# SmoothKen/knn-svc

Measured on AMD Instinct MI355X. Metric: audio-sec converted/sec (xRT) end-to-end, cold target pool, higher is better.
Workload: dtype f32; 1 GPU; north-star point per rank: 30 s source vs 10 min target pool (20 x 30 s), ckpt_type=mix, post_opt_0.2, cold (pool encoded inside the step); seeded random weights of WavLM-Large (6 layers executed) and the 22.9 M-param generator; nq=1500, np_per_rank=30000, wavlm_batch_chunks=32, pipeline_depth=2

## Files before the change

knn_svc_amd/csrc/gemm2_core.h:

```cpp
#pragma once
#include "common.h"

typedef _Float16 f16x8 __attribute__((ext_vector_type(8)));
typedef _Float16 f16x2_t __attribute__((ext_vector_type(2)));
typedef float f32x2_t __attribute__((ext_vector_type(2)));
typedef unsigned g2_u32x4 __attribute__((ext_vector_type(4)));
typedef unsigned g2_u32x2 __attribute__((ext_vector_type(2)));

constexpr float KN_F16X2_A_SCALE = 16.0f;

__device__ __forceinline__ void f16x2_split4(f32x4 v, float scale, g2_u32x2& hi, g2_u32x2& lo) {
    f32x2_t a = {v[0], v[1]}, b = {v[2], v[3]};
    a *= scale; b *= scale;
    const f16x2_t ha = __builtin_convertvector(a, f16x2_t), hb = __builtin_convertvector(b, f16x2_t);
    const f32x2_t ra = a - __builtin_convertvector(ha, f32x2_t), rb = b - __builtin_convertvector(hb, f32x2_t);
    const f16x2_t la = __builtin_convertvector(ra, f16x2_t), lb = __builtin_convertvector(rb, f16x2_t);
    hi = (g2_u32x2){__builtin_bit_cast(unsigned, ha), __builtin_bit_cast(unsigned, hb)};
    lo = (g2_u32x2){__builtin_bit_cast(unsigned, la), __builtin_bit_cast(unsigned, lb)};
}

typedef __attribute__((address_space(3))) char g2_lds_c;
typedef __attribute__((address_space(3))) g2_u32x4 g2_lds_u4;
typedef __attribute__((address_space(3))) g2_u32x2 g2_lds_u2;

#ifdef KN_WHATIF_NOMFMA
#define KN_F16X2_MMA3(C, FA, FB) C[0] += (float)FA[1][0] * (float)FB[0][0] + (float)FA[0][1] * (float)FB[1][1];
#else
#define KN_F16X2_MMA3(C, FA, FB)                                                                               \
    C = __builtin_amdgcn_mfma_f32_32x32x16_f16(FA[1], FB[0], C, 0, 0, 0);               \
    C = __builtin_amdgcn_mfma_f32_32x32x16_f16(FA[0], FB[1], C, 0, 0, 0);                                      \
    C = __builtin_amdgcn_mfma_f32_32x32x16_f16(FA[0], FB[0], C, 0, 0, 0);
#endif
#define KN_F16X2_SLAB_MMA(A, B)                                                                                \
    _Pragma("unroll") for (int ks = 0; ks < 2; ++ks) {                                                        \
        f16x8 fa[TM][2], fb[TN][2];                                                                            \
        _Pragma("unroll") for (int i = 0; i < TM; ++i)                                                        \
            _Pragma("unroll") for (int p = 0; p < 2; ++p)                                                     \
                fa[i][p] = __builtin_bit_cast(f16x8, *(const g2_lds_u4*)(A + i * 32 * PITCH + p * 64 + ks * 32)); \
        _Pragma("unroll") for (int j = 0; j < TN; ++j)                                                        \
            _Pragma("unroll") for (int p = 0; p < 2; ++p)                                                     \
                fb[j][p] = __builtin_bit_cast(f16x8, *(const g2_lds_u4*)(B + j * 32 * PITCH + p * 64 + ks * 32)); \
        _Pragma("unroll") for (int i = 0; i < TM; ++i)                                                        \
            _Pragma("unroll") for (int j = 0; j < TN; ++j) {                                                  \
                f32x16 c = acc[i][j];                                                                          \
                KN_F16X2_MMA3(c, fa[i], fb[j])                                                                 \
                acc[i][j] = c;                                                                                 \
            }                                                                                                  \
    }
#define KN_SPLIT_B_LOAD(RB, SLAB)                                                                              \
    { const int sl_ = SLAB; bload.begin(sl_); _Pragma("unroll") for (int j = 0; j < B_P; ++j) RB[j] = bload(sl_, j, rb_desc); }
#define KN_SPLIT_B_STAGE(RB, BOFF)                                                                             \
    _Pragma("unroll") for (int j = 0; j < B_P; ++j) {                                                         \
        const int q = tid + 256 * j;                                                                          \
        if (B_PIECES % 256 == 0 || q < B_PIECES) *(g2_lds_u4*)(lds + BOFF + (q >> 3) * PITCH + (q & 7) * 16) = RB[j]; \
    }

__host__ __device__ __forceinline__ bool quad_order_swap(long gx, long gy) {
    const long gx8 = (gx + 7) / 8 * 8, gy8 = (gy + 7) / 8 * 8;
    return (gx8 - gx) * 16 > gx8 && (gx8 - gx) * gy8 > (gy8 - gy) * gx8;
}
__host__ __device__ __forceinline__ bool quad_order_linear(long gx, long gy) {
    const long gx8 = (gx + 7) / 8 * 8, gy8 = (gy + 7) / 8 * 8;
    return (gx8 - gx) * 16 > gx8 && (gy8 - gy) * 16 > gy8;
}
__host__ __device__ __forceinline__ long quad_order_ids(long gx, long gy) {
    if (quad_order_linear(gx, gy)) return gx * gy;
    return quad_order_swap(gx, gy) ? (gy + 7) / 8 * 8 * gx : (gx + 7) / 8 * 8 * gy;
}
__device__ __forceinline__ bool quad_order_decode(int L, int gx, int gy, int& mt, int& nt, int rot = 0) {
    if (quad_order_linear(gx, gy)) { mt = L % gx; nt = L / gx; return true; }
    const bool sw = quad_order_swap(gx, gy);
    const int ga = sw ? gy : gx, gb = sw ? gx : gy;
    const int ga8 = (ga + 7) / 8 * 8;
    constexpr int CW = 4;
    const int full = (gb / CW) * CW * ga8;
    int c0, cw;
    if (L < full) { c0 = (L / (CW * ga8)) * CW; cw = CW; L -= (c0 / CW) * CW * ga8; }
    else { c0 = (gb / CW) * CW; cw = gb - c0; L -= full; }
    const int grp = L / (8 * cw), rem = L - grp * 8 * cw;
    const int at = grp * 8 + ((rem + rot) & 7), bt = c0 + (rem >> 3);
    mt = sw ? bt : at; nt = sw ? at : bt;
    return at < ga;
}

__host__ __device__ __forceinline__ bool patch_order_plain(long gx, long gy) { return gy == 1 && gx % 8 != 0; }
__host__ __device__ __forceinline__ long patch_order_ids(long gx, long gy) {
    return (patch_order_plain(gx, gy) ? gx : (gx + 7) / 8 * 8) * gy;
}
template <int BM, int BN>
__device__ __forceinline__ bool patch_order_decode(int plain, int m, int n, int& m0, int& n0) {
    const int gy = (n + BN - 1) / BN;
    const int gx8 = (int)gridDim.x / gy;
    constexpr int CW = 8;
    int L = blockIdx.x;
    const int full = (gy / CW) * CW * gx8;
    int c0, cw;
    if (L < full) { c0 = (L / (CW * gx8)) * CW; cw = CW; L -= (c0 / CW) * CW * gx8; }
    else { c0 = (gy / CW) * CW; cw = gy - c0; L -= full; }
    const int grp = L / (8 * cw), rem = L - grp * 8 * cw;
    m0 = plain ? (int)blockIdx.x * BM : (grp * 8 + ((rem + (int)blockIdx.z) & 7)) * BM;
    n0 = plain ? 0 : (c0 + (rem >> 3)) * BN;
    return m0 < m;
}

#ifdef KN_QUAD_PROF
__device__ long long kn_quad_prof_buf[8192 * 4];
#endif

template <int BM_, int BN_, int WM_, int WN_, int TM_, int TN_>
struct Gemm2Tile : Acc32<WN_, TM_, TN_> {
    typedef f32x16 acc_t;
    static constexpr int NR = 16;
    static constexpr int BM = BM_, BN = BN_, WM = WM_, WN = WN_, TM = TM_, TN = TN_;
    static constexpr int BK = 32, PITCH = 144, THREADS = 256;
    static_assert(WM * WN == 4 && WM * TM * 32 == BM && WN * TN * 32 == BN, "tile shape");
    static constexpr int A_F4 = BM / 32;
    static constexpr int B_PIECES = BN * 8;
    static constexpr int B_P = (B_PIECES + 255) / 256;
    static constexpr int LDS_BYTES = (BM + BN) * PITCH;

    __device__ __forceinline__ static void split_store(g2_lds_c* dst, f32x4 v, float a_scale) {
        g2_u32x2 hi, lo;
        f16x2_split4(v, a_scale, hi, lo);
        *(g2_lds_u2*)(dst) = hi;
        *(g2_lds_u2*)(dst + 64) = lo;
    }

    template <bool A2 = false, class ALoad, class BLoad, class RA, class RB>
    __device__ __forceinline__ static void mainloop(float* lds_generic, int nk, ALoad& aload, BLoad& bload,
                                                    f32x16 (&acc)[TM][TN], RA ra_desc, RB rb_desc, float a_scale) {
        g2_lds_c* lds = (g2_lds_c*)lds_generic;
        const int tid = threadIdx.x;
        const int a_st = (tid >> 3) * PITCH + (tid & 7) * (A2 ? 16 : 8);
        const int lane = tid & 63, wave = tid >> 6;
        const int wm = wave / WN, wn = wave % WN;
        const int li = lane & 31, lh = lane >> 5;
        const int a_frag = (wm * TM * 32 + li) * PITCH + lh * 16;
        const int b_frag = BM * PITCH + (wn * TN * 32 + li) * PITCH + lh * 16;

        f32x4 ra[A_F4];
        g2_u32x4 rb[B_P];
#define KN_STAGE2()                                                                                               \
    {                                                                                                            \
        _Pragma("unroll") for (int j = 0; j < A_F4; ++j) {                                                       \
            if constexpr (A2) *(g2_lds_u4*)(lds + a_st + 32 * j * PITCH) = __builtin_bit_cast(g2_u32x4, ra[j]);   \
            else split_store(lds + a_st + 32 * j * PITCH, aload.finish(ra[j]), a_scale);                         \
        }                                                                                                        \
        KN_SPLIT_B_STAGE(rb, BM * PITCH)                                                                         \
    }
        aload.begin(0); bload.begin(0);
#pragma unroll
        for (int j = 0; j < A_F4; ++j) ra[j] = aload(0, j, ra_desc);
#pragma unroll
        for (int j = 0; j < B_P; ++j) rb[j] = bload(0, j, rb_desc);
        KN_STAGE2();
        __syncthreads();

        for (int kt = 0; kt < nk; ++kt) {
            const bool more = (kt + 1 < nk);
            if (more) {
                aload.begin(kt + 1); bload.begin(kt + 1);
#pragma unroll
                for (int j = 0; j < A_F4; ++j) ra[j] = aload(kt + 1, j, ra_desc);
#pragma unroll
                for (int j = 0; j < B_P; ++j) rb[j] = bload(kt + 1, j, rb_desc);
            }
            KN_F16X2_SLAB_MMA(lds + a_frag, lds + b_frag)
            __syncthreads();
            if (more) KN_STAGE2();
            __syncthreads();
        }
#undef KN_STAGE2
    }
};

struct Gemm2QuadS {
    typedef f32x4 acc_t;
    static constexpr int NR = 4;
    static constexpr int BM = 256, BN = 256, WM = 2, WN = 2, TM = 8, TN = 8;
    static constexpr int EPI_TN = 4;
    static constexpr int ROW = 128, NW = 4, THREADS = 256;
    static constexpr int A_P = BM * ROW / 1024 / NW, B_P = BN * ROW / 1024 / NW;
    static_assert(A_P == 8 && B_P == 8, "schedule below is written for 8 + 8 pieces");
    static constexpr int BOFF = BM * ROW;
    static constexpr int STAGE = (BM + BN) * ROW;
    static constexpr int EPI_BYTES = NW * 32 * (EPI_TN * 32 + 4) * 4;
    static constexpr int LDS_BYTES = 2 * STAGE > EPI_BYTES ? 2 * STAGE : EPI_BYTES;
    static constexpr int OOB_OFF = 0x40000000;

    typedef __attribute__((address_space(3))) char lds_c;
    typedef __attribute__((address_space(3))) g2_u32x4 lds_u4;

    template <class RowOff, class Step, class RA, class RB>
    __device__ __forceinline__ static void mainloop(float* lds_generic, int nk, RowOff a_row_off, Step a_step, RA ra_desc,
                                                    RB rb_desc, int N, int K, int m0, int n0, f32x4 (&acc)[TM][TN]) {
        lds_c* lds = (lds_c*)lds_generic;
        const int tid = threadIdx.x, lane = tid & 63, wave = __builtin_amdgcn_readfirstlane(tid >> 6);
        const int wm = wave / WN, wn = wave % WN;
        const int a_row = (wm * 128 + (lane & 15)) * ROW;
        const int b_row = BOFF + (wn * 128 + (lane & 15)) * ROW;
        int x_off[2];
#pragma unroll
        for (int p = 0; p < 2; ++p) x_off[p] = ((p * 4 + (lane >> 4)) ^ (lane & 7)) * 16;
        int a_src[A_P], b_src[B_P];
        const int row_bytes = (K / 32) * 128;
#pragma unroll
        for (int t = 0; t < A_P; ++t) {
            const int row = (wave * A_P + t) * 8 + (lane >> 3);
            const int ro = a_row_off(m0 + row);
            a_src[t] = ro == OOB_OFF ? OOB_OFF : ro + (lane & 7) * 16;
        }
#pragma unroll
        for (int t = 0; t < B_P; ++t) {
            const int row = (wave * B_P + t) * 8 + (lane >> 3);
            b_src[t] = (n0 + row < N) ? (n0 + row) * row_bytes + (lane & 7) * 16 : OOB_OFF;
        }
        const int st_dst = wave * 8 * 1024 + (lane >> 3) * ROW + (((lane & 7) ^ (lane >> 3)) * 16);
        int ua = 0;
        int a_issued = 0, b_issued = 0;
        g2_u32x4 st[8];
#define KN_S_LOAD_A(T) { st[T] = __builtin_amdgcn_raw_buffer_load_b128(ra_desc, a_src[T] + ua, 0, 0); }
#define KN_S_LOAD_B(T) { st[T] = __builtin_amdgcn_raw_buffer_load_b128(rb_desc, b_src[T], b_issued * 128, 0); }
#define KN_S_WRITE(T, OFF) { *(lds_u4*)(lds + (OFF) + st_dst + (T) * 1024) = st[T]; }
        f16x8 fa[2][4][2], fb[2][4][2];
#define KN_S_READ_A(SET, STG, II, I) { _Pragma("unroll") for (int p = 0; p < 2; ++p) fa[SET][I][p] = __builtin_bit_cast(f16x8, *(const lds_u4*)(lds + (STG) + a_row + ((II) * 4 + (I)) * 16 * ROW + x_off[p])); }
#define KN_S_READ_B(SET, STG, JJ, J) { _Pragma("unroll") for (int p = 0; p < 2; ++p) fb[SET][J][p] = __builtin_bit_cast(f16x8, *(const lds_u4*)(lds + (STG) + b_row + ((JJ) * 4 + (J)) * 16 * ROW + x_off[p])); }
#define KN_S_MFMA1(C, A, B) asm volatile("v_mfma_f32_16x16x32_f16 %0, %1, %2, %0" : "+a"(C) : "v"(A), "v"(B));
#define KN_S_MFMA(AS, BS, I, J)                                                                                           \
    {                                                                                                                     \
        KN_S_MFMA1(acc[(AS) * 4 + (I)][(BS) * 4 + (J)], fa[AS][I][1], fb[BS][J][0])                 \
        KN_S_MFMA1(acc[(AS) * 4 + (I)][(BS) * 4 + (J)], fa[AS][I][0], fb[BS][J][1])                                       \
        KN_S_MFMA1(acc[(AS) * 4 + (I)][(BS) * 4 + (J)], fa[AS][I][0], fb[BS][J][0])                                       \
    }
        ua = a_step(0);
#pragma unroll
        for (int t = 0; t < 8; ++t) KN_S_LOAD_A(t)
        a_issued = 1;
#pragma unroll
        for (int t = 0; t < 8; ++t) KN_S_WRITE(t, 0)
#pragma unroll
        for (int t = 0; t < 8; ++t) KN_S_LOAD_B(t)
        b_issued = 1;
#pragma unroll
        for (int t = 0; t < 8; ++t) KN_S_WRITE(t, BOFF)
        if (nk > 1) {
            ua = a_step(1);
#pragma unroll
            for (int t = 0; t < 8; ++t) KN_S_LOAD_A(t)
            a_issued = 2;
        }
        __builtin_amdgcn_s_waitcnt(0xC07F);
        __builtin_amdgcn_s_barrier();
#ifdef KN_QUAD_PROF
        if (threadIdx.x == 0 && blockIdx.x < 8192) kn_quad_prof_buf[blockIdx.x * 4 + 1] = (long long)__builtin_amdgcn_s_memrealtime();
#endif
#pragma unroll
        for (int i = 0; i < 4; ++i) KN_S_READ_A(0, 0, 0, i)
#pragma unroll
        for (int j = 0; j < 4; ++j) KN_S_READ_B(0, 0, 0, j)

#define KN_S_SLAB(FB, HN, ML)                                                                                             \
    {                                                                                                                     \
        constexpr int cstg = (FB) * STAGE, nstg = (1 - (FB)) * STAGE;              \
                                                                                                     \
        _Pragma("unroll") for (int t = 0; t < 16; ++t) {                                                                  \
            KN_S_MFMA(0, FB, t >> 2, t & 3)                                                                               \
            __builtin_amdgcn_sched_barrier(0);                                                                            \
            if (t < 8) { if (t < 4) KN_S_READ_B(1 - (FB), cstg, 1 - (FB), t) }                                            \
            else if (HN) KN_S_WRITE(t - 8, nstg)                                                                          \
            __builtin_amdgcn_sched_barrier(0);                                                                            \
        }                                                                                                                 \
                                                                                                   \
        _Pragma("unroll") for (int t = 0; t < 16; ++t) {                                                                  \
            KN_S_MFMA(0, 1 - (FB), t >> 2, t & 3)                                                                         \
            __builtin_amdgcn_sched_barrier(0);                                                                            \
            if (t < 8) { if (HN) KN_S_LOAD_B(t) }                                                                         \
            else if (t < 12) KN_S_READ_A(1, cstg, 1, t - 8)                                                               \
            __builtin_amdgcn_sched_barrier(0);                                                                            \
        }                                                                                                                 \
        if (HN) ++b_issued;                                                                                               \
        if (ML) ua = a_step(a_issued);                                                                                    \
                                                                                                   \
        _Pragma("unroll") for (int t = 0; t < 16; ++t) {                                                                  \
            KN_S_MFMA(1, 1 - (FB), t >> 2, t & 3)                                                                         \
            __builtin_amdgcn_sched_barrier(0);                                                                            \
            if (t >= 8) {                                                                                                 \
                if (HN) KN_S_WRITE(t - 8, nstg + BOFF)                                                                    \
                if (ML) KN_S_LOAD_A(t - 8)                                                                                \
            }                                                                                                             \
            __builtin_amdgcn_sched_barrier(0);                                                                            \
        }                                                                                                                 \
        if (ML) ++a_issued;                                                                                               \
        if (HN) { __builtin_amdgcn_s_waitcnt(0xC07F); __builtin_amdgcn_s_barrier(); }                                     \
                     \
        _Pragma("unroll") for (int t = 0; t < 16; ++t) {                                                                  \
            KN_S_MFMA(1, FB, t >> 2, t & 3)                                                                               \
            __builtin_amdgcn_sched_barrier(0);                                                                            \
            if (HN) {                                                                                                     \
                if (t < 4) KN_S_READ_A(0, nstg, 0, t)                                                                     \
                else if (t >= 8 && t < 12) KN_S_READ_B(1 - (FB), nstg, 1 - (FB), t - 8)                                   \
            }                                                                                                             \
            __builtin_amdgcn_sched_barrier(0);                                                                            \
        }                                                                                                                 \
    }
        int s = 0;
        for (; s + 1 < nk; s += 2) {
            KN_S_SLAB(0, true, true)
            KN_S_SLAB(1, true, true)
        }
        if (s < nk) KN_S_SLAB(0, true, true)
#undef KN_S_SLAB
#undef KN_S_MFMA
#undef KN_S_MFMA1
#undef KN_S_READ_A
#undef KN_S_READ_B
#undef KN_S_WRITE
#undef KN_S_LOAD_A
#undef KN_S_LOAD_B
    }

    __device__ __forceinline__ static int acc_row(int wave, int lane, int i, int r) { return (wave / WN) * 128 + i * 16 + 4 * (lane >> 4) + r; }
    __device__ __forceinline__ static int acc_col(int wave, int lane, int j) { return (wave % WN) * 128 + j * 16 + (lane & 15); }

};

template <int BM_, int BN_, int WM_, int WN_, int TM_, int TN_, int HALO_, int DEEP_ = 0>
struct Gemm2Win : Acc32<WN_, TM_, TN_> {
    static constexpr int DEEP = DEEP_;
    typedef f32x16 acc_t;
    static constexpr int NR = 16;
    static constexpr int BM = BM_, BN = BN_, WM = WM_, WN = WN_, TM = TM_, TN = TN_, HALO = HALO_;
    static constexpr int BK = 32, PITCH = 144, THREADS = 256;
    static_assert(WM * WN == 4 && WM * TM * 32 == BM && WN * TN * 32 == BN && HALO % 32 == 0, "tile shape");
    static constexpr int WR = BM + HALO;
    static constexpr int W_F4 = WR / 32;
    static constexpr int B_PIECES = BN * 8;
    static constexpr int B_P = (B_PIECES + 255) / 256;
    static constexpr int BOFF = WR * PITCH;
    static constexpr int LDS_BYTES = (WR + BN) * PITCH;

#define KN_WIN_LOAD(CS)                                                                                        \
    _Pragma("unroll") for (int j = 0; j < W_F4; ++j)                                                          \
        rw[j] = __builtin_bit_cast(f32x4, __builtin_amdgcn_raw_buffer_load_b128(ra_desc, w_off0 + j * 32 * row_bytes + (CS) * 128, 0, 0));
#define KN_WIN_STAGE()                                                                                         \
    _Pragma("unroll") for (int j = 0; j < W_F4; ++j) {                                                        \
        f32x4 v = rw[j];                                                                                      \
        if (a_slope != 1.0f) { _Pragma("unroll") for (int e = 0; e < 4; ++e) v[e] = v[e] > 0.f ? v[e] : v[e] * a_slope; } \
        g2_u32x2 hi, lo;                                                                                      \
        f16x2_split4(v, a_scale, hi, lo);                                                                     \
        *(g2_lds_u2*)(lds + w_st + 32 * j * PITCH) = hi;                                                      \
        *(g2_lds_u2*)(lds + w_st + 32 * j * PITCH + 64) = lo;                                                 \
    }

    template <class BLoad, class RA, class RB>
    __device__ __forceinline__ static void mainloop(float* lds_generic, int ncs, int taps, int dil, int w_off0, int row_bytes,
                                                    BLoad& bload, f32x16 (&acc)[TM][TN], RA ra_desc, RB rb_desc,
                                                    float a_scale, float a_slope) {
        g2_lds_c* lds = (g2_lds_c*)lds_generic;
        const int tid = threadIdx.x;
        const int w_st = (tid >> 3) * PITCH + (tid & 7) * 8;
        const int lane = tid & 63, wave = tid >> 6;
        const int wm = wave / WN, wn = wave % WN;
        const int li = lane & 31, lh = lane >> 5;
        const int a_frag = (wm * TM * 32 + li) * PITCH + lh * 16;
        const int b_frag = BOFF + (wn * TN * 32 + li) * PITCH + lh * 16;
        const int tap_step = dil * PITCH;

        f32x4 rw[W_F4];
        g2_u32x4 rb[B_P];
        KN_WIN_LOAD(0)
        KN_SPLIT_B_LOAD(rb, 0)
        KN_WIN_STAGE()
        KN_SPLIT_B_STAGE(rb, BOFF)
        __syncthreads();
        for (int cs = 0; cs < ncs; ++cs) {
            const bool more_cs = cs + 1 < ncs;
            if (more_cs) { KN_WIN_LOAD(cs + 1) }
            int tap_off = 0;
            for (int tap = 0; tap < taps; ++tap, tap_off += tap_step) {
                const bool last_tap = tap + 1 == taps;
                const bool more = !last_tap || more_cs;
#ifndef KN_WIN_NOBLOAD
                if (more) {
                    const int slab = last_tap ? (cs + 1) : ((tap + 1) * ncs + cs);
                    KN_SPLIT_B_LOAD(rb, slab)
                }
#endif
                KN_F16X2_SLAB_MMA(lds + a_frag + tap_off, lds + b_frag)
#ifndef KN_WIN_NOBAR
                __syncthreads();
#endif
#ifndef KN_WIN_NOBLOAD
                if (more) { KN_SPLIT_B_STAGE(rb, BOFF) }
#endif
                if (last_tap && more_cs) { KN_WIN_STAGE() }
#ifndef KN_WIN_NOBAR
                __syncthreads();
#endif
            }
        }
    }

    template <class BLoad, class RA, class RB>
    __device__ __forceinline__ static void mainloop_deep(float* lds_generic, int ncs, int taps, int dil, int w_off0, int row_bytes,
                                                         BLoad& bload, f32x16 (&acc)[TM][TN], RA ra_desc, RB rb_desc,
                                                         float a_scale, float a_slope) {
        g2_lds_c* lds = (g2_lds_c*)lds_generic;
        const int tid = threadIdx.x;
        const int w_st = (tid >> 3) * PITCH + (tid & 7) * 8;
        const int lane = tid & 63, wave = tid >> 6;
        const int wm = wave / WN, wn = wave % WN;
        const int li = lane & 31, lh = lane >> 5;
        const int a_frag = (wm * TM * 32 + li) * PITCH + lh * 16;
        const int b_frag = BOFF + (wn * TN * 32 + li) * PITCH + lh * 16;
        const int tap_step = dil * PITCH;
        const int nsteps = ncs * taps;
        f32x4 rw[W_F4];
        g2_u32x4 rb[2][B_P];
        auto slab_of = [&](int s) { const int c = s / taps; return (s - c * taps) * ncs + c; };
        KN_WIN_LOAD(0)
        KN_SPLIT_B_LOAD(rb[0], slab_of(0))
        KN_WIN_STAGE()
        KN_SPLIT_B_STAGE(rb[0], BOFF)
        if (nsteps > 1) KN_SPLIT_B_LOAD(rb[1], slab_of(1))
        if (nsteps > 2) KN_SPLIT_B_LOAD(rb[0], slab_of(2))
        __syncthreads();
        int cs = 0, tap = 0, tap_off = 0;
#define KN_D_STEP(SET)                                                                                         \
    {                                                                                                          \
        const bool last_tap = tap + 1 == taps;                                                                 \
        const bool more_cs = cs + 1 < ncs;                                                                     \
        if (tap == 0 && more_cs) { KN_WIN_LOAD(cs + 1) }                                                       \
        KN_F16X2_SLAB_MMA(lds + a_frag + tap_off, lds + b_frag)                                                \
        __syncthreads();                                                                                       \
        if (s + 1 < nsteps) { KN_SPLIT_B_STAGE(rb[SET], BOFF) }                                                \
        if (s + 3 < nsteps) { KN_SPLIT_B_LOAD(rb[SET], slab_of(s + 3)) }                                       \
        if (last_tap && more_cs) { KN_WIN_STAGE() }                                                            \
        __syncthreads();                                                                                       \
        if (last_tap) { tap = 0; tap_off = 0; ++cs; } else { ++tap; tap_off += tap_step; }                     \
    }
        int s = 0;
        for (; s + 1 < nsteps; s += 2) {
            KN_D_STEP(1)
            ++s;
            KN_D_STEP(0)
            --s;
        }
        if (s < nsteps) { KN_D_STEP(1) }
#undef KN_D_STEP
    }
#undef KN_WIN_LOAD
#undef KN_WIN_STAGE

    template <class BLoad, class RB>
    __device__ __forceinline__ static void mainloop_resident(float* lds_generic, int ncs, int taps, int img_slab_bytes, int boff,
                                                             BLoad& bload, f32x16 (&acc)[TM][TN], RB rb_desc) {
        g2_lds_c* lds = (g2_lds_c*)lds_generic;
        const int tid = threadIdx.x;
        const int lane = tid & 63, wave = tid >> 6;
        const int wm = wave / WN, wn = wave % WN;
        const int li = lane & 31, lh = lane >> 5;
        const int a_frag = (wm * TM * 32 + li) * PITCH + lh * 16;
        const int b_frag = boff + (wn * TN * 32 + li) * PITCH + lh * 16;
        g2_u32x4 rb[B_P];
        KN_SPLIT_B_LOAD(rb, 0)
        KN_SPLIT_B_STAGE(rb, boff)
        __syncthreads();
        for (int cs = 0; cs < ncs; ++cs) {
            const bool more_cs = cs + 1 < ncs;
            const int a_cs = a_frag + cs * img_slab_bytes;
            for (int tap = 0; tap < taps; ++tap) {
                const bool last_tap = tap + 1 == taps;
                const bool more = !last_tap || more_cs;
                if (more) {
                    const int slab = last_tap ? (cs + 1) : ((tap + 1) * ncs + cs);
                    KN_SPLIT_B_LOAD(rb, slab)
                }
                KN_F16X2_SLAB_MMA(lds + a_cs + tap * PITCH, lds + b_frag)
                __syncthreads();
                if (more) { KN_SPLIT_B_STAGE(rb, boff) }
                __syncthreads();
            }
        }
    }
};
```

Measured before the change: 924.0 x real-time.

## Use direct buffer-to-LDS loads in quad GEMM mainloop instead of register staging

Replaces the global-load-into-registers then ds_write staging in the Gemm2QuadS mainloop with buffer_load ... lds instructions that write straight into shared memory. The XOR swizzle moves from the LDS destination to the global source offset, and the prefetch schedule and waitcnt/barrier placement are reworked around the new async loads. The aim is to free VGPRs and remove the LDS write instructions from the MFMA-interleaved schedule. In exchange it depends on correct vmcnt accounting and gives up the old per-slab compile-time control flags, which risks races or stalls if the waits are wrong.

```diff
diff --git a/knn_svc_amd/csrc/gemm2_core.h b/knn_svc_amd/csrc/gemm2_core.h
--- a/knn_svc_amd/csrc/gemm2_core.h
+++ b/knn_svc_amd/csrc/gemm2_core.h
@@ -190,6 +190,7 @@
 
     typedef __attribute__((address_space(3))) char lds_c;
     typedef __attribute__((address_space(3))) g2_u32x4 lds_u4;
+    typedef __attribute__((address_space(3))) void lds_v;
 
     template <class RowOff, class Step, class RA, class RB>
     __device__ __forceinline__ static void mainloop(float* lds_generic, int nk, RowOff a_row_off, Step a_step, RA ra_desc,
@@ -204,24 +205,22 @@
         for (int p = 0; p < 2; ++p) x_off[p] = ((p * 4 + (lane >> 4)) ^ (lane & 7)) * 16;
         int a_src[A_P], b_src[B_P];
         const int row_bytes = (K / 32) * 128;
+        const int src_chunk = ((lane & 7) ^ (lane >> 3)) * 16;
 #pragma unroll
         for (int t = 0; t < A_P; ++t) {
             const int row = (wave * A_P + t) * 8 + (lane >> 3);
             const int ro = a_row_off(m0 + row);
-            a_src[t] = ro == OOB_OFF ? OOB_OFF : ro + (lane & 7) * 16;
+            a_src[t] = ro == OOB_OFF ? OOB_OFF : ro + src_chunk;
         }
 #pragma unroll
         for (int t = 0; t < B_P; ++t) {
             const int row = (wave * B_P + t) * 8 + (lane >> 3);
-            b_src[t] = (n0 + row < N) ? (n0 + row) * row_bytes + (lane & 7) * 16 : OOB_OFF;
-        }
-        const int st_dst = wave * 8 * 1024 + (lane >> 3) * ROW + (((lane & 7) ^ (lane >> 3)) * 16);
+            b_src[t] = (n0 + row < N) ? (n0 + row) * row_bytes + src_chunk : OOB_OFF;
+        }
+        lds_c* const st_dst = lds + wave * 8 * 1024;
         int ua = 0;
-        int a_issued = 0, b_issued = 0;
-        g2_u32x4 st[8];
-#define KN_S_LOAD_A(T) { st[T] = __builtin_amdgcn_raw_buffer_load_b128(ra_desc, a_src[T] + ua, 0, 0); }
-#define KN_S_LOAD_B(T) { st[T] = __builtin_amdgcn_raw_buffer_load_b128(rb_desc, b_src[T], b_issued * 128, 0); }
-#define KN_S_WRITE(T, OFF) { *(lds_u4*)(lds + (OFF) + st_dst + (T) * 1024) = st[T]; }
+#define KN_S_DMA_A(T, STG) { __builtin_amdgcn_raw_ptr_buffer_load_lds(ra_desc, (lds_v*)(st_dst + (STG) + (T) * 1024), 16, a_src[T] + ua, 0, 0, 0); }
+#define KN_S_DMA_B(T, STG, SLAB) { __builtin_amdgcn_raw_ptr_buffer_load_lds(rb_desc, (lds_v*)(st_dst + (STG) + BOFF + (T) * 1024), 16, b_src[T], (SLAB) * 128, 0, 0); }
         f16x8 fa[2][4][2], fb[2][4][2];
 #define KN_S_READ_A(SET, STG, II, I) { _Pragma("unroll") for (int p = 0; p < 2; ++p) fa[SET][I][p] = __builtin_bit_cast(f16x8, *(const lds_u4*)(lds + (STG) + a_row + ((II) * 4 + (I)) * 16 * ROW + x_off[p])); }
 #define KN_S_READ_B(SET, STG, JJ, J) { _Pragma("unroll") for (int p = 0; p < 2; ++p) fb[SET][J][p] = __builtin_bit_cast(f16x8, *(const lds_u4*)(lds + (STG) + b_row + ((JJ) * 4 + (J)) * 16 * ROW + x_off[p])); }
@@ -234,22 +233,17 @@
     }
         ua = a_step(0);
 #pragma unroll
-        for (int t = 0; t < 8; ++t) KN_S_LOAD_A(t)
-        a_issued = 1;
-#pragma unroll
-        for (int t = 0; t < 8; ++t) KN_S_WRITE(t, 0)
-#pragma unroll
-        for (int t = 0; t < 8; ++t) KN_S_LOAD_B(t)
-        b_issued = 1;
-#pragma unroll
-        for (int t = 0; t < 8; ++t) KN_S_WRITE(t, BOFF)
+        for (int t = 0; t < 8; ++t) KN_S_DMA_A(t, 0)
+#pragma unroll
+        for (int t = 0; t < 8; ++t) KN_S_DMA_B(t, 0, 0)
         if (nk > 1) {
             ua = a_step(1);
 #pragma unroll
-            for (int t = 0; t < 8; ++t) KN_S_LOAD_A(t)
-            a_issued = 2;
-        }
-        __builtin_amdgcn_s_waitcnt(0xC07F);
+            for (int t = 0; t < 8; ++t) KN_S_DMA_A(t, STAGE)
+            __builtin_amdgcn_s_waitcnt(0x0F78);
+        } else {
+            __builtin_amdgcn_s_waitcnt(0x0F70);
+        }
         __builtin_amdgcn_s_barrier();
 #ifdef KN_QUAD_PROF
         if (threadIdx.x == 0 && blockIdx.x < 8192) kn_quad_prof_buf[blockIdx.x * 4 + 1] = (long long)__builtin_amdgcn_s_memrealtime();
@@ -259,64 +253,57 @@
 #pragma unroll
         for (int j = 0; j < 4; ++j) KN_S_READ_B(0, 0, 0, j)
 
-#define KN_S_SLAB(FB, HN, ML)                                                                                             \
+#define KN_S_SLAB(FB, S)                                                                                                  \
     {                                                                                                                     \
         constexpr int cstg = (FB) * STAGE, nstg = (1 - (FB)) * STAGE;              \
+        const bool hn = (S) + 1 < nk, ml = (S) + 2 < nk;                                                                  \
                                                                                                      \
         _Pragma("unroll") for (int t = 0; t < 16; ++t) {                                                                  \
             KN_S_MFMA(0, FB, t >> 2, t & 3)                                                                               \
             __builtin_amdgcn_sched_barrier(0);                                                                            \
-            if (t < 8) { if (t < 4) KN_S_READ_B(1 - (FB), cstg, 1 - (FB), t) }                                            \
-            else if (HN) KN_S_WRITE(t - 8, nstg)                                                                          \
+            if (t < 4) KN_S_READ_B(1 - (FB), cstg, 1 - (FB), t)                                                           \
+            else if (t < 12) { if (hn) KN_S_DMA_B(t - 4, nstg, (S) + 1) }                                                 \
             __builtin_amdgcn_sched_barrier(0);                                                                            \
         }                                                                                                                 \
                                                                                                    \
         _Pragma("unroll") for (int t = 0; t < 16; ++t) {                                                                  \
             KN_S_MFMA(0, 1 - (FB), t >> 2, t & 3)                                                                         \
             __builtin_amdgcn_sched_barrier(0);                                                                            \
-            if (t < 8) { if (HN) KN_S_LOAD_B(t) }                                                                         \
-            else if (t < 12) KN_S_READ_A(1, cstg, 1, t - 8)                                                               \
+            if (t >= 8 && t < 12) KN_S_READ_A(1, cstg, 1, t - 8)                                                          \
             __builtin_amdgcn_sched_barrier(0);                                                                            \
         }                                                                                                                 \
-        if (HN) ++b_issued;                                                                                               \
-        if (ML) ua = a_step(a_issued);                                                                                    \
                                                                                                    \
         _Pragma("unroll") for (int t = 0; t < 16; ++t) {                                                                  \
             KN_S_MFMA(1, 1 - (FB), t >> 2, t & 3)                                                                         \
             __builtin_amdgcn_sched_barrier(0);                                                                            \
-            if (t >= 8) {                                                                                                 \
-                if (HN) KN_S_WRITE(t - 8, nstg + BOFF)                                                                    \
-                if (ML) KN_S_LOAD_A(t - 8)                                                                                \
-            }                                                                                                             \
-            __builtin_amdgcn_sched_barrier(0);                                                                            \
         }                                                                                                                 \
-        if (ML) ++a_issued;                                                                                               \
-        if (HN) { __builtin_amdgcn_s_waitcnt(0xC07F); __builtin_amdgcn_s_barrier(); }                                     \
+         \
+        __builtin_amdgcn_s_waitcnt(0x0070); __builtin_amdgcn_s_barrier();                                                 \
+        if (ml) ua = a_step((S) + 2);                                                                                     \
                      \
         _Pragma("unroll") for (int t = 0; t < 16; ++t) {                                                                  \
             KN_S_MFMA(1, FB, t >> 2, t & 3)                                                                               \
             __builtin_amdgcn_sched_barrier(0);                                                                            \
-            if (HN) {                                                                                                     \
-                if (t < 4) KN_S_READ_A(0, nstg, 0, t)                                                                     \
-                else if (t >= 8 && t < 12) KN_S_READ_B(1 - (FB), nstg, 1 - (FB), t - 8)                                   \
-            }                                                                                                             \
+            if (t < 4) KN_S_READ_A(0, nstg, 0, t)                                                                         \
+            else if (t >= 8 && t < 12) KN_S_READ_B(1 - (FB), nstg, 1 - (FB), t - 8)                                       \
+            else if (ml) KN_S_DMA_A((t < 8 ? t - 4 : t - 8), cstg)                                                        \
             __builtin_amdgcn_sched_barrier(0);                                                                            \
         }                                                                                                                 \
     }
         int s = 0;
         for (; s + 1 < nk; s += 2) {
-            KN_S_SLAB(0, true, true)
-            KN_S_SLAB(1, true, true)
-        }
-        if (s < nk) KN_S_SLAB(0, true, true)
+            KN_S_SLAB(0, s)
+            KN_S_SLAB(1, s + 1)
+        }
+        if (s < nk) KN_S_SLAB(0, s)
+        __builtin_amdgcn_s_waitcnt(0x0F70);
 #undef KN_S_SLAB
 #undef KN_S_MFMA
 #undef KN_S_MFMA1
 #undef KN_S_READ_A
 #undef KN_S_READ_B
-#undef KN_S_WRITE
-#undef KN_S_LOAD_A
-#undef KN_S_LOAD_B
+#undef KN_S_DMA_A
+#undef KN_S_DMA_B
     }
 
     __device__ __forceinline__ static int acc_row(int wave, int lane, int i, int r) { return (wave / WN) * 128 + i * 16 + 4 * (lane >> 4) + r; }
```

After: 929.3 x real-time, median of 6. No clear change (+0.6%).
